# linyicheng1/keypoint_bench

Measured on AMD Instinct MI355X. Metric: image-pairs/sec (extract+NMS+BF-match, 640x480, top_k=1000), higher is better.
Workload: dtype f32

## Files before the change

### keypoint_bench_amd/csrc/alike.hip

```cpp
#include "conv_mfma.h"

namespace {

typedef _Float16 h8v __attribute__((ext_vector_type(8)));
typedef _Float16 h2v __attribute__((ext_vector_type(2)));
typedef float f32x4v __attribute__((ext_vector_type(4)));

__device__ __forceinline__ float relu(float v);

__device__ __forceinline__ void split4(const float4 v, uint2& hi, uint2& lo) { cm_split4(v, hi, lo); }

__device__ __forceinline__ void amax_commit(float lane_max, float* slots, int slot, int lane)
{
    const float m = cm_wave_max(lane_max);
    if (lane == 0) slots[slot] = m;
}

__global__ __launch_bounds__(256) void amax_reduce(const float* slots, int n, unsigned* out)
{
    __shared__ float s[4];
    const int b = blockIdx.x, tid = threadIdx.x;
    float m = 0.0f;
    for (int i = tid; i < n; i += 256) {
        const float v = slots[(size_t)b * n + i];
// ... 452 lines not shown
                    const float4 q = *reinterpret_cast<const float4*>(p + ((size_t)dy * Wr + dx) * CDS + c4 * 4);
                    v4.x = fmaxf(v4.x, q.x); v4.y = fmaxf(v4.y, q.y); v4.z = fmaxf(v4.z, q.z); v4.w = fmaxf(v4.w, q.w);
                }
            const float v[4] = {v4.x, v4.y, v4.z, v4.w};
#pragma unroll
            for (int c = 0; c < 4; ++c)
#pragma unroll
                for (int j = 0; j < 16; ++j) acc[j] = fmaf(v[c], dw[(c4 * 4 + c) * COUT + j], acc[j]);
        }
    }
    float* o = a.out + ((size_t)b * a.H * a.W + (size_t)gy * a.W + gx) * COUT + cg * 16;
#pragma unroll
    for (int q = 0; q < 4; ++q) {
        float4 v = make_float4(acc[4 * q], acc[4 * q + 1], acc[4 * q + 2], acc[4 * q + 3]);
        if (RELU) { v.x = relu(v.x); v.y = relu(v.y); v.z = relu(v.z); v.w = relu(v.w); }
        *reinterpret_cast<float4*>(o + 4 * q) = v;
    }
}

struct Block2Args {
    const float* p1;
    float* x2; float* a2; float* S2;
    float* p2;
    const uint4* w1pk;
    const uint4* w2pk;
    const uint4* wapk;
    const float* b1; const float* bsum; const float* wsg;
    int H, W;
    float inv_ws1, inv_ws2, inv_wsa, l1_c1, bmax_c1, l1_c2, l1_ds, bmax_sum;
    const unsigned* amax_x1;
    float* wmax_a2;
    int xcd_map;
};


__global__ __launch_bounds__(256, 4) void alike_block2(Block2Args a)
{
    constexpr int TH = 8, TW = 32, PH = TH + 4, PW = TW + 4, NP = PH * PW, MH = TH + 2, MW = TW + 2, NM = MH * MW;
    __shared__ __attribute__((aligned(16))) uint4 pin[2 * NP];
    __shared__ __attribute__((aligned(16))) uint4 mid[4 * NM];
    __shared__ __attribute__((aligned(16))) uint4 xs[4][2][2][16];
    __shared__ __attribute__((aligned(16))) uint4 zslot;
    const kpb_tile3 tile = kpb_xcd_tile(a.xcd_map);
    const int tid = threadIdx.x, lane = tid & 63, wv = tid >> 6, b = tile.z;
    const int ty0 = tile.y * TH, tx0 = tile.x * TW;
    const size_t P = (size_t)a.H * a.W;
    h8v w1h[3], w1l[3], w2h[5], w2l[5];
#pragma unroll
    for (int kb = 0; kb < 3; ++kb) { w1h[kb] = __builtin_bit_cast(h8v, a.w1pk[(kb * 2) * 64 + lane]); w1l[kb] = __builtin_bit_cast(h8v, a.w1pk[(kb * 2 + 1) * 64 + lane]); }
    const float4 b1v = *reinterpret_cast<const float4*>(a.b1 + 4 * (lane >> 4));
    const float4 bsum = *reinterpret_cast<const float4*>(a.bsum + 4 * (lane >> 4)), wsg = *reinterpret_cast<const float4*>(a.wsg + 4 * (lane >> 4));
    const float am_p = __uint_as_float(a.amax_x1[b]);
    const float bound1 = fmaf(am_p, a.l1_c1, a.bmax_c1);
    const int e1 = cm_exp_of(fmaxf(am_p, bound1));
    const int ex = cm_exp_of(fmaf(bound1, a.l1_c2, fmaf(am_p, a.l1_ds, a.bmax_sum)));
    const float sc1 = cm_scale_of(e1), un_c1s = a.inv_ws1, un_c2 = a.inv_ws2 * cm_unscale_of(e1);
    const bool edge = ty0 == 0 || tx0 == 0 || ty0 + TH >= a.H || tx0 + TW >= a.W;
    const float scx = cm_scale_of(ex), un_a = a.inv_wsa * cm_unscale_of(ex);
    {
        const float* in = a.p1 + (size_t)b * P * 8;
        constexpr int PER = (NP * 2 + 255) / 256;
        float4 ld[PER];
        unsigned okm = 0;
#pragma unroll
        for (int k = 0; k < PER; ++k) {
            const int i = min(tid + 256 * k, NP * 2 - 1);
            const int pos = i >> 1, q = i & 1;
            const int y = pos / PW, x = pos - y * PW;
            const int gy = ty0 - 2 + y, gx = tx0 - 2 + x;
            if (gy >= 0 && gy < a.H && gx >= 0 && gx < a.W) okm |= 1u << k;
            ld[k] = *reinterpret_cast<const float4*>(in + ((size_t)min(max(gy, 0), a.H - 1) * a.W + min(max(gx, 0), a.W - 1)) * 8 + 4 * q);
        }
#pragma unroll
        for (int k = 0; k < PER; ++k) {
            const int i = tid + 256 * k;
            const int pos = i >> 1, q = i & 1;
            float4 v = ((okm >> k) & 1u) ? ld[k] : make_float4(0.f, 0.f, 0.f, 0.f);
            v.x *= sc1; v.y *= sc1; v.z *= sc1; v.w *= sc1;
            uint2 hi, lo;
            split4(v, hi, lo);
            if (i < NP * 2) {
                uint2* d = reinterpret_cast<uint2*>(&pin[pos]) + q;
                d[0] = hi;
                d[2 * NP] = lo;
            }
        }
        if (tid == 0) zslot = make_uint4(0u, 0u, 0u, 0u);
    }
    __syncthreads();
    const int px = lane & 15, g = lane >> 4;
    const uint4* zp = &zslot;
    {
        float4 bias1 = b1v;
        bias1.x *= sc1; bias1.y *= sc1; bias1.z *= sc1; bias1.w *= sc1;
        uint2* midh = reinterpret_cast<uint2*>(mid);
        static_assert((2 * MH) % 4 == 0, "alike_block2: the regular conv1 groups split evenly over the four waves");
        {
            const int xl = 16 * (wv & 1) + px, y0 = wv >> 1;
            const int gxl = tx0 - 1 + xl;
            const bool xin = gxl >= 0 && gxl < a.W;
            const float unm = xin ? un_c1s : 0.0f;
            const float4 bm = xin ? bias1 : make_float4(0.f, 0.f, 0.f, 0.f);
            const bool has2 = 8 + g < 9;
            const uint4* q0 = &pin[(y0 + g / 3) * PW + xl + g % 3];
            const uint4* q1 = &pin[(y0 + (4 + g) / 3) * PW + xl + (4 + g) % 3];
            const uint4* q2 = has2 ? &pin[(y0 + 2) * PW + xl + 2] : zp;
            const int st2 = has2 ? 2 * PW : 0, lo2 = has2 ? NP : 0;
            int h8 = (((g >> 1) * NM + y0 * MW + xl) << 1) + (g & 1);
            constexpr int NIT = 2 * MH / 4;
            h8v i0h = __builtin_bit_cast(h8v, q0[0]), i0l = __builtin_bit_cast(h8v, q0[NP]);
            h8v i1h = __builtin_bit_cast(h8v, q1[0]), i1l = __builtin_bit_cast(h8v, q1[NP]);
            h8v i2h = __builtin_bit_cast(h8v, q2[0]), i2l = __builtin_bit_cast(h8v, q2[lo2]);
#pragma unroll 1
            for (int it = 0; it < NIT; ++it, h8 += 4 * MW) {
                f32x4v acc = {0.f, 0.f, 0.f, 0.f};
                __builtin_amdgcn_sched_barrier(0);
                acc = __builtin_amdgcn_mfma_f32_16x16x32_f16(w1h[0], i0l, acc, 0, 0, 0);
                acc = __builtin_amdgcn_mfma_f32_16x16x32_f16(w1l[0], i0h, acc, 0, 0, 0);
                acc = __builtin_amdgcn_mfma_f32_16x16x32_f16(w1h[0], i0h, acc, 0, 0, 0);
                acc = __builtin_amdgcn_mfma_f32_16x16x32_f16(w1h[1], i1l, acc, 0, 0, 0);
                acc = __builtin_amdgcn_mfma_f32_16x16x32_f16(w1l[1], i1h, acc, 0, 0, 0);
                acc = __builtin_amdgcn_mfma_f32_16x16x32_f16(w1h[1], i1h, acc, 0, 0, 0);
                acc = __builtin_amdgcn_mfma_f32_16x16x32_f16(w1h[2], i2l, acc, 0, 0, 0);
                acc = __builtin_amdgcn_mfma_f32_16x16x32_f16(w1l[2], i2h, acc, 0, 0, 0);
                acc = __builtin_amdgcn_mfma_f32_16x16x32_f16(w1h[2], i2h, acc, 0, 0, 0);
                __builtin_amdgcn_sched_barrier(0);
                if (it + 1 < NIT) {
                    q0 += 2 * PW; q1 += 2 * PW; q2 += st2;
                    i0h = __builtin_bit_cast(h8v, q0[0]); i0l = __builtin_bit_cast(h8v, q0[NP]);
                    i1h = __builtin_bit_cast(h8v, q1[0]); i1l = __builtin_bit_cast(h8v, q1[NP]);
                    i2h = __builtin_bit_cast(h8v, q2[0]); i2l = __builtin_bit_cast(h8v, q2[lo2]);
                }
                __builtin_amdgcn_sched_barrier(0);
                const bool yin = (unsigned)(ty0 - 1 + y0 + 2 * it) < (unsigned)a.H;
                float4 v = make_float4(0.f, 0.f, 0.f, 0.f);
                if (yin) v = make_float4(relu(fmaf(acc[0], unm, bm.x)), relu(fmaf(acc[1], unm, bm.y)), relu(fmaf(acc[2], unm, bm.z)), relu(fmaf(acc[3], unm, bm.w)));
                uint2 hi, lo;
                split4(v, hi, lo);
                midh[h8] = hi;
                midh[h8 + 4 * NM] = lo;
            }
        }
        if (wv < 2) {
            const int gi = 2 * MH + wv;
            const int k = 16 * (gi - 2 * MH) + px;
            const int y = k >> 1, x = 32 + (k & 1);
            const int my = min(y, MH - 1);
            f32x4v acc = {0.f, 0.f, 0.f, 0.f};
#pragma unroll
            for (int kb = 0; kb < 3; ++kb) {
                const int tap = 4 * kb + g;
                const bool has = tap < 9;
                const uint4* ph = has ? &pin[(my + tap / 3) * PW + x + tap % 3] : zp;
                const h8v ihi = __builtin_bit_cast(h8v, ph[0]);
                const h8v ilo = __builtin_bit_cast(h8v, has ? ph[NP] : zp[0]);
                acc = __builtin_amdgcn_mfma_f32_16x16x32_f16(w1h[kb], ilo, acc, 0, 0, 0);
                acc = __builtin_amdgcn_mfma_f32_16x16x32_f16(w1l[kb], ihi, acc, 0, 0, 0);
                acc = __builtin_amdgcn_mfma_f32_16x16x32_f16(w1h[kb], ihi, acc, 0, 0, 0);
            }
            const int gy = ty0 - 1 + y, gx = tx0 - 1 + x;
            const bool inside = gy >= 0 && gy < a.H && gx >= 0 && gx < a.W;
            float4 v = make_float4(relu(fmaf(acc[0], un_c1s, bias1.x)), relu(fmaf(acc[1], un_c1s, bias1.y)), relu(fmaf(acc[2], un_c1s, bias1.z)), relu(fmaf(acc[3], un_c1s, bias1.w)));
            if (edge && !inside) v = make_float4(0.f, 0.f, 0.f, 0.f);
            uint2 hi, lo;
            split4(v, hi, lo);
            if (y < MH) {
                const int h8 = (((g >> 1) * NM + y * MW + x) << 1) + (g & 1);
                midh[h8] = hi;
                midh[h8 + 4 * NM] = lo;
            }
        }
    }
    __builtin_amdgcn_sched_barrier(0);
#pragma unroll
    for (int kb = 0; kb < 5; ++kb) { w2h[kb] = __builtin_bit_cast(h8v, a.w2pk[(kb * 2) * 64 + lane]); w2l[kb] = __builtin_bit_cast(h8v, a.w2pk[(kb * 2 + 1) * 64 + lane]); }
    const h8v wah = __builtin_bit_cast(h8v, a.wapk[lane]), wal = __builtin_bit_cast(h8v, a.wapk[64 + lane]);
    __syncthreads();
    float* x2 = a.x2 + (size_t)b * P * 16;
    float* a2 = a.a2 + (size_t)b * P * 16;
    float* S2 = a.S2 + (size_t)b * P;
    uint2* xh = reinterpret_cast<uint2*>(&xs[wv][0][0][0]);
    float4 pm = make_float4(0.f, 0.f, 0.f, 0.f);
    float amx = 0.0f;
#pragma unroll 1
    for (int k4 = 0; k4 < 4; ++k4) {
        const int row = 4 * (wv >> 1) + k4, col0 = (wv & 1) * 16;
        const int mbase = row * MW + col0 + px;
        f32x4v acc = {0.f, 0.f, 0.f, 0.f};
        h8v ihi[5], ilo[5];
        auto fetch = [&](int kb) {
            const int kidx = 4 * kb + g;
            const uint4* ph;
            int lo_off;
            if (kidx < 18) { const int tap = kidx >> 1; ph = &mid[(kidx & 1) * NM + mbase + (tap / 3) * MW + tap % 3]; lo_off = 2 * NM; }
            else if (kidx == 18) { ph = &pin[(row + 2) * PW + col0 + px + 2]; lo_off = NP; }
            else { ph = zp; lo_off = 0; }
            ihi[kb] = __builtin_bit_cast(h8v, ph[0]);
            ilo[kb] = __builtin_bit_cast(h8v, ph[lo_off]);
        };
        auto mm = [&](int kb) {
            acc = __builtin_amdgcn_mfma_f32_16x16x32_f16(w2h[kb], ilo[kb], acc, 0, 0, 0);
            acc = __builtin_amdgcn_mfma_f32_16x16x32_f16(w2l[kb], ihi[kb], acc, 0, 0, 0);
            acc = __builtin_amdgcn_mfma_f32_16x16x32_f16(w2h[kb], ihi[kb], acc, 0, 0, 0);
        };
        fetch(0); fetch(1); fetch(2);
        __builtin_amdgcn_sched_barrier(0);
        mm(0); mm(1);
        __builtin_amdgcn_sched_barrier(0);
        fetch(3); fetch(4);
        __builtin_amdgcn_sched_barrier(0);
        mm(2);
        __builtin_amdgcn_sched_barrier(0);
        mm(3); mm(4);
        const int gy = ty0 + row, gx = tx0 + col0 + px;
        const bool ok = gy < a.H && gx < a.W;
        const float4 v = make_float4(relu(fmaf(acc[0], un_c2, bsum.x)), relu(fmaf(acc[1], un_c2, bsum.y)), relu(fmaf(acc[2], un_c2, bsum.z)), relu(fmaf(acc[3], un_c2, bsum.w)));
        if (ok && !a.p2) *reinterpret_cast<float4*>(x2 + ((size_t)gy * a.W + gx) * 16 + 4 * g) = v;
        pm = make_float4(kpb_pmax(pm.x, v.x), kpb_pmax(pm.y, v.y), kpb_pmax(pm.z, v.z), kpb_pmax(pm.w, v.w));
        {
            uint2 hi, lo;
            split4(make_float4(v.x * scx, v.y * scx, v.z * scx, v.w * scx), hi, lo);
            const int h8 = (((g >> 1) * 16 + px) << 1) + (g & 1);
            xh[h8] = hi;
            xh[h8 + 64] = lo;
        }
        f32x4v ag = {0.f, 0.f, 0.f, 0.f};
        {
            const uint4* ph = g < 2 ? &xs[wv][0][g][px] : zp;
            const h8v ihi = __builtin_bit_cast(h8v, ph[0]);
            const h8v ilo = __builtin_bit_cast(h8v, g < 2 ? ph[32] : zp[0]);
            ag = __builtin_amdgcn_mfma_f32_16x16x32_f16(wah, ilo, ag, 0, 0, 0);
            ag = __builtin_amdgcn_mfma_f32_16x16x32_f16(wal, ihi, ag, 0, 0, 0);
            ag = __builtin_amdgcn_mfma_f32_16x16x32_f16(wah, ihi, ag, 0, 0, 0);
        }
        const float4 av = make_float4(relu(ag[0] * un_a), relu(ag[1] * un_a), relu(ag[2] * un_a), relu(ag[3] * un_a));
        if (ok) {
            *reinterpret_cast<float4*>(a2 + ((size_t)gy * a.W + gx) * 16 + 4 * g) = av;
            amx = kpb_pmax(kpb_pmax(amx, kpb_pmax(av.x, av.y)), kpb_pmax(av.z, av.w));
        }
        float sg = fmaf(av.w, wsg.w, fmaf(av.z, wsg.z, fmaf(av.y, wsg.y, av.x * wsg.x)));
        sg = kpb_sum16(sg);
        sg = kpb_sum32(sg);
        if (g == 0 && ok) S2[(size_t)gy * a.W + gx] = sg;
    }
    if (a.p2) {
        pm.x = kpb_pmax(pm.x, kpb_xor1(pm.x)); pm.y = kpb_pmax(pm.y, kpb_xor1(pm.y));
        pm.z = kpb_pmax(pm.z, kpb_xor1(pm.z)); pm.w = kpb_pmax(pm.w, kpb_xor1(pm.w));
        pm.x = kpb_pmax(pm.x, kpb_xor2(pm.x)); pm.y = kpb_pmax(pm.y, kpb_xor2(pm.y));
        pm.z = kpb_pmax(pm.z, kpb_xor2(pm.z)); pm.w = kpb_pmax(pm.w, kpb_xor2(pm.w));
        const int gy = ty0 + 4 * (wv >> 1), gx = tx0 + (wv & 1) * 16 + px;
        if ((px & 3) == 0 && gy < a.H && gx < a.W)
            *reinterpret_cast<float4*>(a.p2 + (size_t)b * (P / 16) * 16 + ((size_t)(gy >> 2) * (a.W >> 2) + (gx >> 2)) * 16 + 4 * g) = pm;
    }
    amax_commit(amx, a.wmax_a2, ((b * gridDim.y + tile.y) * gridDim.x + tile.x) * 4 + wv, lane);
}

std::vector<float> pack_1x1_h16(const float* w, float scale)
{
    return pack_lanes_h16(1, [&](int, int l, int j) {
        const int n = l & 15, g = l >> 4;
        return g < 2 ? w[n * 16 + 8 * g + j] * scale : 0.0f;
    });
}

std::vector<float> pack_h16(const float* w, int CIN, const float* ds_w, float scale)
{
    const int OCT = CIN / 8, NK = 9 * OCT + (ds_w ? 1 : 0), KB = (NK + 3) / 4;
    return pack_lanes_h16(KB, [&](int kb, int l, int j) {
        const int n = l & 15, g = l >> 4, kidx = 4 * kb + g;
        float v = 0.0f;
        if (kidx < 9 * OCT) { const int tap = kidx / OCT, o = kidx - tap * OCT; v = w[((size_t)n * CIN + 8 * o + j) * 9 + tap]; }
        else if (ds_w && kidx == 9 * OCT) v = ds_w[n * 8 + j];
        return v * scale;
    });
}

// ... 35 lines not shown
    if (STAGE_IN) {
        const int ln = threadIdx.x & 63;
        const size_t pw = (size_t)bx * 256 + (threadIdx.x >> 6) * 64;
        float4 ld[CIN / 4];
#pragma unroll
        for (int i = 0; i < CIN / 4; ++i) {
            const int j = ln + 64 * i, px = j / (CIN / 4);
            ld[i] = pw + px < npix ? *reinterpret_cast<const float4*>(in + pw * CIN + 4 * (size_t)j) : make_float4(0.f, 0.f, 0.f, 0.f);
        }
#pragma unroll
        for (int i = 0; i < CIN / 4; ++i) {
            const int j = ln + 64 * i, px = j / (CIN / 4), q = j - px * (CIN / 4);
            *reinterpret_cast<float4*>(wreg + px * XP + 4 * q) = ld[i];
        }
        x = wreg + ln * XP;
    }
#pragma unroll 2
    for (int c4 = 0; c4 < CIN / 4; ++c4) {
        const float4 v4 = *reinterpret_cast<const float4*>(x + c4 * 4);
        const float v[4] = {v4.x, v4.y, v4.z, v4.w};
#pragma unroll
        for (int c = 0; c < 4; ++c)
#pragma unroll
            for (int j = 0; j < 16; ++j) acc[j] = fmaf(v[c], w[(c4 * 4 + c) * 16 + j], acc[j]);
    }
    float sg = 0.0f;
#pragma unroll
    for (int j = 0; j < 16; ++j) { acc[j] = relu(acc[j]); sg = fmaf(acc[j], wsg[j], sg); }
    if (live) {
        float* o = out + p * 16;
#pragma unroll
        for (int q = 0; q < 4; ++q)
            *reinterpret_cast<float4*>(o + 4 * q) = make_float4(acc[4 * q], acc[4 * q + 1], acc[4 * q + 2], acc[4 * q + 3]);
        smap[p] = sg;
    }
    if (E) {
        const int lane = threadIdx.x & 63, wv = threadIdx.x >> 6;
        float* st = wreg;
        const size_t p0 = (size_t)bx * 256 + wv * 64;
        float4 r[17];
#pragma unroll
        for (int q = 0; q < 16; ++q) {
            r[q] = make_float4(0.f, 0.f, 0.f, 0.f);
#pragma unroll
            for (int c = 0; c < 16; ++c) {
                const float* wr = wproj + c * 64 + 4 * q;
                r[q].x = fmaf(acc[c], wr[0], r[q].x); r[q].y = fmaf(acc[c], wr[1], r[q].y);
                r[q].z = fmaf(acc[c], wr[2], r[q].z); r[q].w = fmaf(acc[c], wr[3], r[q].w);
            }
        }
        r[16] = make_float4(sg, 0.f, 0.f, 0.f);
        for (int g = 0; g < 4; ++g) {
            if ((lane >> 4) == g) {
                float* e = st + (lane & 15) * ESTRIDE;
#pragma unroll
                for (int q = 0; q < 17; ++q) *reinterpret_cast<float4*>(e + 4 * q) = r[q];
            }
            const size_t base = p0 + 16 * g;
            for (int j = lane; j < 16 * (ESTRIDE / 4); j += 64)
                if (base + j / (ESTRIDE / 4) < npix)
                    *reinterpret_cast<float4*>(E + base * ESTRIDE + 4 * j) = *reinterpret_cast<const float4*>(st + 4 * j);
        }
    }
}

template <int CIN>
__global__ __launch_bounds__(256) void conv1x1_relu(const float* __restrict__ in, float* __restrict__ out, const float* __restrict__ w,
// ... 954 lines not shown
#pragma unroll
            for (int k = 0; k < 3; ++k) ds[r * (GP_TW * 3) + lane * 3 + k] = __fdiv_rn(1.0f, 1.0f + expf(-z[k]));
        }
    }
    if (!a.desc) return;
    __builtin_amdgcn_wave_barrier();
    const int vw = min(GP_TW, W - tx0) * 3;
#pragma unroll
    for (int k = 0; k < GP_RPT * GP_TW * 3 / 4 / 64; ++k) {
        const int f = k * 64 + lane, r = f / (GP_TW * 3 / 4), c4 = (f - r * (GP_TW * 3 / 4)) * 4;
        if (c4 < vw && yw + r < H)
            *reinterpret_cast<float4*>(a.desc + (img + (size_t)(yw + r) * W + tx0) * 3 + c4) = *reinterpret_cast<const float4*>(ds + r * (GP_TW * 3) + c4);
    }
}

}

namespace {

struct AlikeBlock1 : kpb_net {
    float* x1 = nullptr;
    struct { const float *w1, *b1, *w2, *b2; const uint4 *w1pk, *w2pk; float inv_ws1, inv_ws2, l1_c1, bmax_c1; } k1 = {};
    struct B1Bufs { float *p1, *wmax_x1; unsigned* amax_x1; };
    static int b1_waves(int H, int W) { return cdiv(W, B1_TW) * cdiv(H, B1H_TH) * 4; }
    void block1(const float* img_dev, int batch, int H, int W, const B1Bufs& b);
};

struct AlikeTrunk : AlikeBlock1 {
    float *a2 = nullptr, *a3 = nullptr, *a4 = nullptr;
    struct { const uint4 *w1pk, *w2pk, *wapk; const float *b1, *bsum; float inv_ws1, inv_ws2, inv_wsa, l1_c1, bmax_c1, l1_c2, l1_ds, bmax_sum; } k2 = {};
    struct Res { const float *w1, *b1, *w2, *b2, *dsw, *dsb, *w1h, *b1h, *w2p, *b2p; float un1, un2; const char *prof1, *prof2; } blk[5] = {};
    struct { const float *agg[5], *whT, *wsc; const uint4 *wh16, *a1h16; float l1_agg1, inv_ws_h, inv_wa; } kh = {};
    struct Maps { float *S2, *S3, *S4, *E3, *E4; unsigned *amax_x1, *amax_a2; };
    int trunk(const float* img_dev, int batch, int H, int W, bool dense, Maps& m);
};

struct AlikeNet : AlikeTrunk {
    int forward(const float* img_dev, int batch, int H_, int W_, float* score_out_dev, float* desc_out_dev) override;
    int desc_at(const float* pts_dev, int pts_cols, int max_n, const int32_t* n_dev, float* out_dev) override;
};

void repack3x3(const float* w, int co, int ci, std::vector<float>& out)
{
    out.resize((size_t)9 * ci * co);
    for (int o = 0; o < co; ++o)
        for (int c = 0; c < ci; ++c)
            for (int k = 0; k < 9; ++k) out[((size_t)k * ci + c) * co + o] = w[((size_t)o * ci + c) * 9 + k];
}
void transpose(const float* w, int co, int ci, std::vector<float>& out)
{
    out.resize((size_t)ci * co);
    for (int o = 0; o < co; ++o)
        for (int c = 0; c < ci; ++c) out[(size_t)c * co + o] = w[(size_t)o * ci + c];
}
float l1_rows(const float* w, int co, int per)
{
    float m = 0.0f;
    for (int o = 0; o < co; ++o) {
        double s = 0.0;
        for (int i = 0; i < per; ++i) s += std::fabs((double)w[(size_t)o * per + i]);
        m = std::max(m, (float)(s * (1.0 + 1e-6)));
    }
    return m;
}
float max_abs(const float* b, int n)
{
    float m = 0.0f;
// ... 16 lines not shown
__global__ __launch_bounds__(256) void maxpool4_nhwc(const float* __restrict__ in, float* __restrict__ out, int Ho, int Wo, int C)
{
    const int C4 = C / 4;
    const size_t i = (size_t)blockIdx.x * 256 + threadIdx.x, b = blockIdx.y;
    if (i >= (size_t)Ho * Wo * C4) return;
    const int c = (int)(i % C4) * 4;
    const size_t pix = i / C4;
    const int y = (int)(pix / Wo), x = (int)(pix - (size_t)y * Wo);
    const float* s = in + ((b * 4 * Ho + 4 * y) * (size_t)(4 * Wo) + 4 * x) * C + c;
    float4 m = *reinterpret_cast<const float4*>(s);
#pragma unroll
    for (int py = 0; py < 4; ++py)
#pragma unroll
        for (int px = 0; px < 4; ++px) {
            if (py == 0 && px == 0) continue;
            const float4 v = *reinterpret_cast<const float4*>(s + ((size_t)py * 4 * Wo + px) * C);
            m.x = fmaxf(m.x, v.x); m.y = fmaxf(m.y, v.y); m.z = fmaxf(m.z, v.z); m.w = fmaxf(m.w, v.w);
        }
    *reinterpret_cast<float4*>(out + ((b * Ho + y) * (size_t)Wo + x) * C + c) = m;
}

void AlikeBlock1::block1(const float* img_dev, int batch, int H, int W, const B1Bufs& b)
{
    hipStream_t st = ctx->stream;
    Block1Args b1{img_dev, x1, b.p1, k1.w1, k1.b1, k1.w2, k1.b2, H, W};
    if (conv_mfma_use_h16()) {
        Block1HArgs hb{b1, k1.w1pk, k1.w2pk, k1.inv_ws1, k1.inv_ws2, k1.l1_c1, k1.bmax_c1, b.wmax_x1, 0};
        KPB_LAUNCH(ctx, "alike_block1", alike_block1_h, dim3(cdiv(W, B1_TW), cdiv(H, B1H_TH), batch), dim3(256), 0, st, hb);
        KPB_LAUNCH(ctx, "amax_reduce", amax_reduce, dim3(batch), dim3(256), 0, st, b.wmax_x1, b1_waves(H, W), b.amax_x1);
    } else
        KPB_LAUNCH(ctx, "alike_block1", alike_block1, dim3(cdiv(W, B1_TW), cdiv(H, B1_TH), batch), dim3(256), 0, st, b1);
}

int AlikeTrunk::trunk(const float* img_dev, int batch, int H, int W, bool dense, Maps& mo)
{
    const size_t P = (size_t)H * W, B = batch;
    const bool h16 = conv_mfma_use_h16();
    const bool fused = h16 && batch >= 16 && ctx->alike_coarse_fused;
    const int nw1 = b1_waves(H, W), nw2 = cdiv(W / 2, 32) * cdiv(H / 2, 8) * 4;
    const size_t n_2 = B * (P / 4) * 16, n_3 = B * (P / 64) * 32, n_4 = B * (P / 1024) * 64;
    float *p1, *t2, *x2, *t3, *x3, *t4, *x4, *r3, *r4, *t3r3, *t4r4, *p2, *p3, *S2, *S3, *S4, *E3, *E4, *wmax_x1, *wmax_a2;
    unsigned *amax_x1, *amax_a2;
    if (int rc = kpb_carve(ctx, act, [&](Arena& a) {
            auto f32 = [&](size_t n) { return h16 ? nullptr : a.take(n); };
            auto f16 = [&](size_t n) { return h16 ? a.take(n) : nullptr; };
            x1 = a.take(B * P * 8);
            p1 = a.take(B * (P / 4) * 8);
            t2 = f32(n_2); x2 = f32(n_2); a2 = a.take(n_2);
            t3 = f32(n_3); x3 = fused ? nullptr : a.take(n_3); a3 = a.take(B * (P / 64) * 16);
            t4 = f32(n_4); x4 = fused ? nullptr : a.take(n_4); a4 = a.take(B * (P / 1024) * 16);
            r3 = f32(n_3); r4 = f32(n_4);
            t3r3 = f16(2 * n_3);
            t4r4 = f16(2 * n_4);
            p2 = f16(n_3 / 2);
            p3 = h16 && batch >= 16 ? a.take(n_4 / 2) : nullptr;
            S2 = a.take(B * (P / 4)); S3 = a.take(B * (P / 64)); S4 = a.take(B * (P / 1024));
            E3 = dense ? a.take(B * (P / 64) * ESTRIDE) : nullptr;
            E4 = dense ? a.take(B * (P / 1024) * ESTRIDE) : nullptr;
            amax_x1 = h16 ? a.take<unsigned>(B) : nullptr;
            amax_a2 = h16 ? a.take<unsigned>(B) : nullptr;
            wmax_x1 = f16(B * nw1);
            wmax_a2 = f16(B * nw2);
        }))
        return rc;
    this->B = batch; this->H = H; this->W = W;
    hipStream_t st = ctx->stream;

    block1(img_dev, batch, H, W, B1Bufs{p1, wmax_x1, amax_x1});
    ConvArgs c;
    if (h16) {
        Block2Args b2{p1, x2, a2, S2, p2, k2.w1pk, k2.w2pk, k2.wapk, k2.b1, k2.bsum, kh.wsc + 16, H / 2, W / 2,
                      k2.inv_ws1, k2.inv_ws2, k2.inv_wsa, k2.l1_c1, k2.bmax_c1, k2.l1_c2, k2.l1_ds, k2.bmax_sum, amax_x1, wmax_a2, 1};
        KPB_LAUNCH(ctx, "alike_block2", alike_block2, dim3(cdiv(W / 2, 32), cdiv(H / 2, 8), batch), dim3(256), 0, st, b2);
        KPB_LAUNCH(ctx, "amax_reduce", amax_reduce, dim3(batch), dim3(256), 0, st, wmax_a2, nw2, amax_a2);
        auto block_h = [&](const Res& r, const float* in, float* tr, float* xo, int cin, int cout, int Hi, int Wi, bool prepooled, int gi = 0, float* ao = nullptr,
                           float* So = nullptr, float* Eo = nullptr, float* pool = nullptr) {
            ConvM m{.in = in, .out = tr, .wp = r.w1h, .bias = r.b1h, .Hi = prepooled ? Hi / 4 : Hi, .Wi = prepooled ? Wi / 4 : Wi,
                    .H = Hi / 4, .W = Wi / 4, .CIN = cin, .COUT = 2 * cout, .NCH = 1, .relu = 2, .nblk = cout / 32, .istride = cin, .ostride = 2 * cout,
                    .unscale = r.un1, .relu_nt = cout / 32};
            auto launch = [&](const char* prof, const CmForm& f, const ConvM& cm) {
                return launch_conv_mfma_h<CM_C16, CM_C32, CM_C32_1T, CM_C16_LAT, CM_C32_LAT, CM_P4_LAT, CM_B3C2_TAIL, CM_B4C2_TAIL>(ctx, prof, f, cm, batch); };
            if (batch < 16 && !prepooled) m.nblk = 2 * cout / 32;
            const CmForm f1 = !prepooled ? CM_P4_LAT : batch < 16 ? CM_C16_LAT : cin == 32 ? CM_C32 : CM_C16;
            if (int rc = launch(r.prof1, f1, m)) return rc;
            ConvM c2{.in = tr, .out = xo, .wp = r.w2p, .bias = r.b2p, .res = tr + cout, .Hi = Hi / 4, .Wi = Wi / 4,
                     .H = Hi / 4, .W = Wi / 4, .CIN = cout, .COUT = cout, .NCH = cout / 32, .nblk = batch < 16 ? cout / 32 : 1, .istride = 2 * cout,
                     .ostride = cout, .unscale = r.un2, .rstride = 2 * cout};
            if (ao) {
                c2.tl_w = kh.agg[gi]; c2.tl_wsg = kh.wsc + 16 * (gi - 1); c2.tl_wproj = kh.whT + 16 * (gi - 1) * 64;
                c2.tl_agg = ao; c2.tl_smap = So; c2.tl_E = Eo; c2.tl_pool = pool;
                return launch(r.prof2, pool ? CM_B3C2_TAIL : CM_B4C2_TAIL, c2);
            }
            return launch(r.prof2, batch < 16 ? CM_C32_LAT : cout == 32 ? CM_C32_1T : CM_C32, c2);
        };
        if (fused) {
            if (int rc = block_h(blk[3], p2, t3r3, nullptr, 16, 32, H / 2, W / 2, true, 3, a3, S3, E3, p3)) return rc;
            if (int rc = block_h(blk[4], p3, t4r4, nullptr, 32, 64, H / 8, W / 8, true, 4, a4, S4, E4)) return rc;
        } else if (int rc = block_h(blk[3], p2, t3r3, x3, 16, 32, H / 2, W / 2, true))
            return rc;
        else if (batch >= 16) {
            KPB_LAUNCH(ctx, "maxpool4_x3", maxpool4_nhwc, dim3((unsigned)(((size_t)(H / 32) * (W / 32) * 8 + 255) / 256), batch), dim3(256), 0, st, x3, p3, H / 32, W / 32, 32);
            if (int rc = block_h(blk[4], p3, t4r4, x4, 32, 64, H / 8, W / 8, true)) return rc;
        } else if (int rc = block_h(blk[4], x3, t4r4, x4, 32, 64, H / 8, W / 8, false))
            return rc;
    } else {
        auto conv2 = [&](const Res& r, const float* in, float* out, const float* res, int h, int w, int c) {
// ... 7 lines not shown
        c = ConvArgs{t2, x2, blk[2].w2, blk[2].b2, p1, blk[2].dsw, blk[2].dsb, nullptr, H / 2, W / 2};
        launch_conv<16, 16, 1, true, 8, 1>(ctx, "conv3x3_b2c2", st, c, batch);
        c = ConvArgs{x2, t3, blk[3].w1, blk[3].b1, nullptr, blk[3].dsw, blk[3].dsb, r3, H / 8, W / 8};
        launch_conv<16, 32, 4, false, 4, 1, true, 16>(ctx, "conv3x3_b3c1", st, c, batch);
        if (int rc = conv2(blk[3], t3, x3, r3, H / 8, W / 8, 32)) return rc;
        c = ConvArgs{x3, t4, blk[4].w1, blk[4].b1, nullptr, blk[4].dsw, blk[4].dsb, r4, H / 32, W / 32};
        launch_conv<32, 64, 4, false, 4, 1, true, 16>(ctx, "conv3x3_b4c1", st, c, batch);
        if (int rc = conv2(blk[4], t4, x4, r4, H / 32, W / 32, 64)) return rc;
        KPB_LAUNCH(ctx, "conv1x1_agg2", conv1x1_relu<16>, dim3((unsigned)((B * P / 4 + 255) / 256)), dim3(256), 0, st, x2, a2, kh.agg[2], kh.wsc + 16, S2, B * P / 4, nullptr, nullptr);
    }
    if (fused)
        ;
    else if (batch < 16) {
        const AggArgs g3{x3, a3, kh.agg[3], kh.wsc + 32, S3, B * P / 64, kh.whT + 32 * 64, E3};
        const AggArgs g4{x4, a4, kh.agg[4], kh.wsc + 48, S4, B * P / 1024, kh.whT + 48 * 64, E4};
        const unsigned nb3 = (unsigned)((B * P / 64 + 255) / 256), nb4 = (unsigned)((B * P / 1024 + 255) / 256);
        KPB_LAUNCH(ctx, "conv1x1_agg34", conv1x1_relu_34, dim3(nb3 + nb4), dim3(256), 0, st, g3, g4, nb3);
    } else {
        KPB_LAUNCH(ctx, "conv1x1_agg3", conv1x1_relu<32>, dim3((unsigned)((B * P / 64 + 255) / 256)), dim3(256), 0, st, x3, a3, kh.agg[3], kh.wsc + 32, S3, B * P / 64, kh.whT + 32 * 64, E3);
        KPB_LAUNCH(ctx, "conv1x1_agg4", conv1x1_relu<64>, dim3((unsigned)((B * P / 1024 + 255) / 256)), dim3(256), 0, st, x4, a4, kh.agg[4], kh.wsc + 48, S4, B * P / 1024, kh.whT + 48 * 64, E4);
    }
    mo = Maps{S2, S3, S4, E3, E4, amax_x1, amax_a2};
    return KPB_OK;
}

int AlikeNet::forward(const float* img_dev, int batch, int H_, int W_, float* score_out_dev, float* desc_out_dev)
{
    if ((H_ % 32) || (W_ % 32))
        return kpb_fail(ctx, KPB_E_INVALID, "kpb_net_forward: ALIKE needs H and W multiples of 32 (got %dx%d)", H_, W_);
    const int H = H_, W = W_;
    const bool h16 = conv_mfma_use_h16();
    const bool dense = desc_out_dev != nullptr;
    Maps m;
    if (int rc = trunk(img_dev, batch, H, W, dense, m)) return rc;
    float *S2 = m.S2, *S3 = m.S3, *S4 = m.S4, *E3 = m.E3, *E4 = m.E4;
    unsigned *amax_x1 = m.amax_x1, *amax_a2 = m.amax_a2;
    hipStream_t st = ctx->stream;
    if (dense) {
        HybArgs hy{x1, a2, E3, E4, kh.agg[1], kh.whT, kh.wsc, score_out_dev, desc_out_dev, H, W, amax_x1, amax_a2, 0.f, 1.f, 1.f, nullptr, 1.f};
        const int work4 = cdiv(H, 4) * cdiv(W / 32, SEG_TILES);
        if (h16) {
            hy.l1_agg1 = kh.l1_agg1; hy.inv_ws_h = kh.inv_ws_h; hy.ws_h = 1.0f / hy.inv_ws_h;
            hy.a1h16 = kh.a1h16; hy.inv_wa = kh.inv_wa;
            if (!hp_ring_rows_ok(H, H / 2, HP_A2R) || !hp_ring_rows_ok(H, H / 8, HP_ER) || !hp_ring_rows_ok(H, H / 32, HP_ER))
                return kpb_fail(ctx, KPB_E_UNSUPPORTED, "alike head: the LDS rings cannot hold the source rows of %d row groups at height %d", HP_LA + 1, H);
            const int bands_ = cdiv(W / 32, HP_TILES), groups_ = H / 4;
            const int hp = std::max(2, std::min(30, (int)(((long long)bands_ * groups_ * batch) / 1536)));
            KPB_LAUNCH(ctx, "alike_head_dense", alike_head_f16p, dim3(cdiv(W / 32, HP_TILES) * cdiv(H / 4, hp), batch), dim3(256), 0, st, hy,
                       kh.wh16, hp);
        } else
            KPB_LAUNCH(ctx, "alike_head_dense", alike_head_hyb, dim3(work4, batch), dim3(256), 0, st, hy);
    } else {
        LinArgs la{x1, S2, S3, S4, kh.agg[1], kh.wsc, score_out_dev, H, W,
                   (float)(H / 2 - 1) / (float)(H - 1), (float)(W / 2 - 1) / (float)(W - 1), (float)(H / 8 - 1) / (float)(H - 1), (float)(W / 8 - 1) / (float)(W - 1),
                   (float)(H / 32 - 1) / (float)(H - 1), (float)(W / 32 - 1) / (float)(W - 1)};
        KPB_LAUNCH(ctx, "alike_head_score", alike_score_lin, dim3(cdiv(H * W, 256), batch), dim3(256), 0, st, la);
    }
    KPB_HIP(ctx, hipGetLastError());
    return KPB_OK;
}

int AlikeNet::desc_at(const float* pts_dev, int pts_cols, int max_n, const int32_t* n_dev, float* out_dev)
{
    if (B == 0) return kpb_fail(ctx, KPB_E_INVALID, "kpb_net_desc_at: no forward has run");
    const int kpw = (long long)B * max_n >= 32768 ? 8 : 1;
    DescAtArgs a{HeadArgs{x1, a2, a3, a4, kh.agg[1], kh.whT, kh.wsc, nullptr, nullptr, H, W}, pts_dev, n_dev, out_dev, pts_cols, max_n, kpw};
    KPB_LAUNCH(ctx, "alike_desc_at", alike_desc_at, dim3(cdiv(max_n, 4 * kpw), B), dim3(256), 0, ctx->stream, a);
// ... 132 lines not shown
    trunk_stage(bl, ws, net.get());
    net->kh.l1_agg1 = l1_rows(bl.get("agg1.w", {dim / 4, c1}), 16, 8);
    const float* hw = bl.get("head.w", {dim + 1, dim});
    transpose(hw, 64, 64, tmp); ws.put(tmp, &net->kh.whT);
    ws.put_raw(hw + 64 * 64, 64, &net->kh.wsc);
    float hmax = 0.0f;
    for (int o = 0; o < 64; ++o) for (int cc = 0; cc < 32; ++cc) hmax = std::max(hmax, std::fabs(hw[o * 64 + cc]));
    const float* a1w = bl.get("agg1.w", {dim / 4, c1});
    const float sh = weight_scale_h(&hmax, 1), sa1 = weight_scale_h(a1w, 16 * 8);
    net->kh.inv_ws_h = 1.0f / sh; net->kh.inv_wa = 1.0f / sa1;
    ws.put(pack_head_h16(hw, sh), &net->kh.wh16);
    ws.put(pack_agg1_h16(a1w, sa1), &net->kh.a1h16);
    if (int rc = ws.upload(ctx, &net->wdev)) return rc;
    *out = net.release();
    return KPB_OK;
}

namespace {

struct EdgePointNet : AlikeTrunk {
    struct { const float *wsc, *tab, *tabb; } ke = {};
    int forward(const float* img_dev, int batch, int H_, int W_, float* score_out_dev, float* desc_out_dev) override;
};

int EdgePointNet::forward(const float* img_dev, int batch, int H_, int W_, float* score_out_dev, float* desc_out_dev)
{
    if ((H_ % 32) || (W_ % 32))
        return kpb_fail(ctx, KPB_E_INVALID, "kpb_net_forward: EdgePoint needs H and W multiples of 32 (got %dx%d)", H_, W_);
    const size_t npix = (size_t)batch * H_ * W_;
    const size_t nb_score = (npix + 256 * EPS_PPL - 1) / (256 * EPS_PPL);
    if (npix / 64 > 0xffffffffu || nb_score > 0x7fffffffu)
        return kpb_fail(ctx, KPB_E_UNSUPPORTED, "kpb_net_forward: EdgePoint: %d images of %dx%d exceed the head kernels' index range", batch, H_, W_);
    Maps m;
    if (int rc = trunk(img_dev, batch, H_, W_, false, m)) return rc;
    hipStream_t st = ctx->stream;
    KPB_LAUNCH(ctx, "edgepoint_score", edgepoint_score, dim3((unsigned)nb_score), dim3(256), 0, st, x1, score_out_dev, ke.wsc, npix);
    if (desc_out_dev) {
        const unsigned nc = (unsigned)(npix / 64);
        EpDescArgs d{x1, a2, a3, a4, ke.wsc, ke.tab, ke.tabb, kh.whT, desc_out_dev, H_, W_, nc};
        KPB_LAUNCH(ctx, "edgepoint_desc", edgepoint_desc, dim3(std::min((nc + 15u) / 16u, 2048u)), dim3(256), 0, st, d);
    }
    KPB_HIP(ctx, hipGetLastError());
    return KPB_OK;
}

}

int edgepoint_create(kpb_ctx* ctx, const KpbwBlob& bl, kpb_net** out)
{
    const uint32_t q = dim / 4;
    if (const char* n = first_missing(bl, {{"head.w", {dim, dim}}, {"score.w", {q}}, {"score.b", {1}}, {"d8.w", {q, q}}, {"d8.b", {q}}, {"d4.w", {q, q}}, {"d4.b", {q}},
                                           {"ct4.w", {q, q, 4, 4}}, {"ct4.b", {q}}}))
        return kpb_fail(ctx, KPB_E_WEIGHTS, "kpb_net_create: tensor %s missing or not EdgePoint shaped "
                        "(this build supports c1..c4 = 8,16,32,64, dim = 64, single head)", n);
    auto net = std::make_unique<EdgePointNet>();
    net->ctx = ctx; net->arch = KPB_ARCH_EDGEPOINT; net->dim = dim; net->desc_div = 8;
    WeightStage ws;
    std::vector<float> tmp;
    trunk_stage(bl, ws, net.get());
    ws.put(std::vector<float>(64, 0.0f), &net->kh.wsc);
    transpose(bl.get("head.w", {dim, dim}), 64, 64, tmp); ws.put(tmp, &net->kh.whT);
    {
        const float *w1 = bl.get("agg1.w", {q, c1}), *wsr = bl.get("score.w", {q});
        tmp.assign(EP_WBIAS + 1, 0.0f);
        for (int c = 0; c < 16; ++c) {
            for (int k = 0; k < 8; ++k) tmp[c * EP_WROW + k] = w1[c * 8 + k];
            tmp[c * EP_WROW + 8] = wsr[c];
// ... 139 lines not shown
```

### keypoint_bench_amd/csrc/conv_mfma.h

```cpp
#pragma once
#include <type_traits>
#include "net.h"

#include <algorithm>
#include <cmath>
#include <cstring>

namespace {

typedef float f32x16 __attribute__((ext_vector_type(16)));

__device__ __forceinline__ float relu(float v) { return fmaxf(v, 0.0f); }

struct ConvM {
    const float* in = nullptr;
    float* out = nullptr;
    const float* wp = nullptr;
    const float* bias = nullptr;
    const float* xf = nullptr;
    const int* active = nullptr;
    const float* res = nullptr;
    int Hi = 0, Wi = 0, H = 0, W = 0, CIN = 0, COUT = 0, NCH = 0, relu = 0, nblk = 0;
    int istride = 0, ostride = 0, ooff = 0;
    float unscale = 1.0f;
// ... 242 lines not shown

template <int CT>
__device__ __forceinline__ void cm_tail_agg(const float* x, float* strip, const float* w_ , const float* wsg_ ,
                                            const float* wproj_ , float* __restrict__ out, float* __restrict__ smap, float* __restrict__ E,
                                            const size_t (&row_pix)[4], const int (&ncol)[4], int lane, int half)
{
    typedef const __attribute__((address_space(4))) float* cfp;
    const cfp w = (cfp)w_, wsg = (cfp)wsg_, wproj = (cfp)wproj_;
    float acc[16];
#pragma unroll
    for (int j = 0; j < 16; ++j) acc[j] = 0.0f;
#pragma unroll 2
    for (int c4 = 0; c4 < CT / 4; ++c4) {
        const float4 v4 = *reinterpret_cast<const float4*>(x + c4 * 4);
        const float v[4] = {v4.x, v4.y, v4.z, v4.w};
#pragma unroll
        for (int c = 0; c < 4; ++c)
#pragma unroll
            for (int j = 0; j < 16; ++j) acc[j] = fmaf(v[c], w[(c4 * 4 + c) * 16 + j], acc[j]);
    }
    float sg = 0.0f;
#pragma unroll
    for (int j = 0; j < 16; ++j) { acc[j] = relu(acc[j]); sg = fmaf(acc[j], wsg[j], sg); }
    const int g_own = lane >> 4, col = lane & 15;
    size_t pix = 0; bool live = false;
#pragma unroll
    for (int g = 0; g < 4; ++g)
        if (g == g_own) { pix = row_pix[g] + col; live = col < ncol[g]; }
    if (live && half == 0) {
        float* o = out + pix * 16;
#pragma unroll
        for (int q = 0; q < 4; ++q)
            *reinterpret_cast<float4*>(o + 4 * q) = make_float4(acc[4 * q], acc[4 * q + 1], acc[4 * q + 2], acc[4 * q + 3]);
        smap[pix] = sg;
    }
    if (!E) return;
#pragma unroll
    for (int rnd = 0; rnd < 2; ++rnd) {
        const int q0 = 8 * half + 4 * rnd;
        float4 r[4];
#pragma unroll
        for (int k = 0; k < 4; ++k) {
            r[k] = make_float4(0.f, 0.f, 0.f, 0.f);
#pragma unroll
            for (int c = 0; c < 16; ++c) {
                const cfp wr = wproj + c * 64 + 4 * (q0 + k);
                r[k].x = fmaf(acc[c], wr[0], r[k].x); r[k].y = fmaf(acc[c], wr[1], r[k].y);
                r[k].z = fmaf(acc[c], wr[2], r[k].z); r[k].w = fmaf(acc[c], wr[3], r[k].w);
            }
        }
#pragma unroll
        for (int g = 0; g < 4; ++g) {
            if (g_own == g) {
#pragma unroll
                for (int k = 0; k < 4; ++k) *reinterpret_cast<float4*>(strip + col * 16 + 4 * k) = r[k];
            }
            if ((lane >> 2) < ncol[g])
                *reinterpret_cast<float4*>(E + (row_pix[g] + (lane >> 2)) * CM_ESTRIDE + 4 * (q0 + (lane & 3))) = *reinterpret_cast<const float4*>(strip + 4 * lane);
        }
    }
    if (live && half == 1) *reinterpret_cast<float4*>(E + pix * CM_ESTRIDE + 64) = make_float4(sg, 0.f, 0.f, 0.f);
}

template <CmForm F>
__global__ __launch_bounds__(256, F.waves()) void conv_mfma_h(ConvM a)
{
    constexpr int KS = F.ks, S = F.s, CC = F.cc, NTB = F.ntb, MT = F.mt, PF = F.pf, WN = F.wn, DIL = F.dil;
// ... 882 lines not shown
```

Measured before the change: 15950.

## Template alike_block2 to skip unused x2 and score-map outputs

alike_block2 becomes a template on whether it writes the x2 map and the per-pixel score map S2. The trunk now allocates and writes S2/S3/S4 only when the share path needs them, which is when no dense descriptors are requested. The x2 store is removed at compile time. Indexing is simplified to a 32-bit pixel offset with column-only bounds, and the conv2 tap fetch now uses a strength-reduced pointer, which relies on new checks that H and W are multiples of 32. Downstream smap writes are guarded by null checks.

Result: no change. 15920 (-0.2%).

```diff
diff --git a/keypoint_bench_amd/csrc/alike.hip b/keypoint_bench_amd/csrc/alike.hip
--- a/keypoint_bench_amd/csrc/alike.hip
+++ b/keypoint_bench_amd/csrc/alike.hip
@@ -508,8 +508,9 @@
     float* wmax_a2;
     int xcd_map;
 };
-
-
+struct B2Form { bool share, x2; };
+
+template <B2Form F>
 __global__ __launch_bounds__(256, 4) void alike_block2(Block2Args a)
 {
     constexpr int TH = 8, TW = 32, PH = TH + 4, PW = TW + 4, NP = PH * PW, MH = TH + 2, MW = TW + 2, NM = MH * MW;
@@ -566,6 +567,7 @@
     __syncthreads();
     const int px = lane & 15, g = lane >> 4;
     const uint4* zp = &zslot;
+    const int wvs = __builtin_amdgcn_readfirstlane(wv);
     {
         float4 bias1 = b1v;
         bias1.x *= sc1; bias1.y *= sc1; bias1.z *= sc1; bias1.w *= sc1;
@@ -608,7 +610,7 @@
                     i2h = __builtin_bit_cast(h8v, q2[0]); i2l = __builtin_bit_cast(h8v, q2[lo2]);
                 }
                 __builtin_amdgcn_sched_barrier(0);
-                const bool yin = (unsigned)(ty0 - 1 + y0 + 2 * it) < (unsigned)a.H;
+                const bool yin = (unsigned)(ty0 - 1 + (wvs >> 1) + 2 * it) < (unsigned)a.H;
                 float4 v = make_float4(0.f, 0.f, 0.f, 0.f);
                 if (yin) v = make_float4(relu(fmaf(acc[0], unm, bm.x)), relu(fmaf(acc[1], unm, bm.y)), relu(fmaf(acc[2], unm, bm.z)), relu(fmaf(acc[3], unm, bm.w)));
                 uint2 hi, lo;
@@ -652,27 +654,33 @@
     for (int kb = 0; kb < 5; ++kb) { w2h[kb] = __builtin_bit_cast(h8v, a.w2pk[(kb * 2) * 64 + lane]); w2l[kb] = __builtin_bit_cast(h8v, a.w2pk[(kb * 2 + 1) * 64 + lane]); }
     const h8v wah = __builtin_bit_cast(h8v, a.wapk[lane]), wal = __builtin_bit_cast(h8v, a.wapk[64 + lane]);
     __syncthreads();
-    float* x2 = a.x2 + (size_t)b * P * 16;
-    float* a2 = a.a2 + (size_t)b * P * 16;
-    float* S2 = a.S2 + (size_t)b * P;
+    char* x2 = F.x2 ? reinterpret_cast<char*>(a.x2 + (size_t)b * P * 16) : nullptr;
+    char* a2 = reinterpret_cast<char*>(a.a2 + (size_t)b * P * 16);
+    char* S2 = F.share ? reinterpret_cast<char*>(a.S2 + (size_t)b * P) : nullptr;
     uint2* xh = reinterpret_cast<uint2*>(&xs[wv][0][0][0]);
     float4 pm = make_float4(0.f, 0.f, 0.f, 0.f);
     float amx = 0.0f;
+    const int row0 = 4 * (wvs >> 1), col0 = (wvs & 1) * 16;
+    const bool colin = tx0 + col0 < a.W;
+    unsigned pixo = (unsigned)((ty0 + row0) * a.W + tx0 + col0 + px);
+    const uint4* q4 = g < 2 ? &mid[g * NM + (row0 + 2) * MW + col0 + px + 2] : g == 2 ? &pin[(row0 + 2) * PW + col0 + px + 2] : zp;
+    const int st4 = g < 2 ? MW : g == 2 ? PW : 0, lo4 = g < 2 ? 2 * NM : g == 2 ? NP : 0;
 #pragma unroll 1
-    for (int k4 = 0; k4 < 4; ++k4) {
-        const int row = 4 * (wv >> 1) + k4, col0 = (wv & 1) * 16;
-        const int mbase = row * MW + col0 + px;
+    for (int k4 = 0; k4 < 4; ++k4, q4 += st4, pixo += (unsigned)a.W) {
+        const int mbase = (row0 + k4) * MW + col0 + px;
         f32x4v acc = {0.f, 0.f, 0.f, 0.f};
         h8v ihi[5], ilo[5];
         auto fetch = [&](int kb) {
-            const int kidx = 4 * kb + g;
-            const uint4* ph;
-            int lo_off;
-            if (kidx < 18) { const int tap = kidx >> 1; ph = &mid[(kidx & 1) * NM + mbase + (tap / 3) * MW + tap % 3]; lo_off = 2 * NM; }
-            else if (kidx == 18) { ph = &pin[(row + 2) * PW + col0 + px + 2]; lo_off = NP; }
-            else { ph = zp; lo_off = 0; }
+            if (kb == 4) {
+                ihi[kb] = __builtin_bit_cast(h8v, q4[0]);
+                ilo[kb] = __builtin_bit_cast(h8v, q4[lo4]);
+                return;
+            }
+            const int kidx = 4 * kb + g, tap = kidx >> 1;
+            const int ty = (tap * 11) >> 5;
+            const uint4* ph = &mid[(kidx & 1) * NM + mbase + ty * MW + tap - 3 * ty];
             ihi[kb] = __builtin_bit_cast(h8v, ph[0]);
-            ilo[kb] = __builtin_bit_cast(h8v, ph[lo_off]);
+            ilo[kb] = __builtin_bit_cast(h8v, ph[2 * NM]);
         };
         auto mm = [&](int kb) {
             acc = __builtin_amdgcn_mfma_f32_16x16x32_f16(w2h[kb], ilo[kb], acc, 0, 0, 0);
@@ -688,10 +696,9 @@
         mm(2);
         __builtin_amdgcn_sched_barrier(0);
         mm(3); mm(4);
-        const int gy = ty0 + row, gx = tx0 + col0 + px;
-        const bool ok = gy < a.H && gx < a.W;
+        const unsigned vo = pixo * 64u + 16u * g;
         const float4 v = make_float4(relu(fmaf(acc[0], un_c2, bsum.x)), relu(fmaf(acc[1], un_c2, bsum.y)), relu(fmaf(acc[2], un_c2, bsum.z)), relu(fmaf(acc[3], un_c2, bsum.w)));
-        if (ok && !a.p2) *reinterpret_cast<float4*>(x2 + ((size_t)gy * a.W + gx) * 16 + 4 * g) = v;
+        if (F.x2 && colin) *reinterpret_cast<float4*>(x2 + vo) = v;
         pm = make_float4(kpb_pmax(pm.x, v.x), kpb_pmax(pm.y, v.y), kpb_pmax(pm.z, v.z), kpb_pmax(pm.w, v.w));
         {
             uint2 hi, lo;
@@ -710,14 +717,16 @@
             ag = __builtin_amdgcn_mfma_f32_16x16x32_f16(wah, ihi, ag, 0, 0, 0);
         }
         const float4 av = make_float4(relu(ag[0] * un_a), relu(ag[1] * un_a), relu(ag[2] * un_a), relu(ag[3] * un_a));
-        if (ok) {
-            *reinterpret_cast<float4*>(a2 + ((size_t)gy * a.W + gx) * 16 + 4 * g) = av;
+        if (colin) {
+            *reinterpret_cast<float4*>(a2 + vo) = av;
             amx = kpb_pmax(kpb_pmax(amx, kpb_pmax(av.x, av.y)), kpb_pmax(av.z, av.w));
         }
-        float sg = fmaf(av.w, wsg.w, fmaf(av.z, wsg.z, fmaf(av.y, wsg.y, av.x * wsg.x)));
-        sg = kpb_sum16(sg);
-        sg = kpb_sum32(sg);
-        if (g == 0 && ok) S2[(size_t)gy * a.W + gx] = sg;
+        if (F.share) {
+            float sg = fmaf(av.w, wsg.w, fmaf(av.z, wsg.z, fmaf(av.y, wsg.y, av.x * wsg.x)));
+            sg = kpb_sum16(sg);
+            sg = kpb_sum32(sg);
+            if (g == 0 && colin) *reinterpret_cast<float*>(S2 + pixo * 4u) = sg;
+        }
     }
     if (a.p2) {
         pm.x = kpb_pmax(pm.x, kpb_xor1(pm.x)); pm.y = kpb_pmax(pm.y, kpb_xor1(pm.y));
@@ -819,7 +828,7 @@
 #pragma unroll
         for (int q = 0; q < 4; ++q)
             *reinterpret_cast<float4*>(o + 4 * q) = make_float4(acc[4 * q], acc[4 * q + 1], acc[4 * q + 2], acc[4 * q + 3]);
-        smap[p] = sg;
+        if (smap) smap[p] = sg;
     }
     if (E) {
         const int lane = threadIdx.x & 63, wv = threadIdx.x >> 6;
@@ -1840,7 +1849,7 @@
     struct Res { const float *w1, *b1, *w2, *b2, *dsw, *dsb, *w1h, *b1h, *w2p, *b2p; float un1, un2; const char *prof1, *prof2; } blk[5] = {};
     struct { const float *agg[5], *whT, *wsc; const uint4 *wh16, *a1h16; float l1_agg1, inv_ws_h, inv_wa; } kh = {};
     struct Maps { float *S2, *S3, *S4, *E3, *E4; unsigned *amax_x1, *amax_a2; };
-    int trunk(const float* img_dev, int batch, int H, int W, bool dense, Maps& m);
+    int trunk(const float* img_dev, int batch, int H, int W, bool dense, bool share, Maps& m);
 };
 
 struct AlikeNet : AlikeTrunk {
@@ -1923,8 +1932,12 @@
         KPB_LAUNCH(ctx, "alike_block1", alike_block1, dim3(cdiv(W, B1_TW), cdiv(H, B1_TH), batch), dim3(256), 0, st, b1);
 }
 
-int AlikeTrunk::trunk(const float* img_dev, int batch, int H, int W, bool dense, Maps& mo)
-{
+int AlikeTrunk::trunk(const float* img_dev, int batch, int H, int W, bool dense, bool share, Maps& mo)
+{
+    if ((H % 32) || (W % 32))
+        return kpb_fail(ctx, KPB_E_INVALID, "alike trunk: H and W must be multiples of 32 (got %dx%d)", H, W);
+    if ((size_t)(H / 2) * (W / 2) * 64 >= ((size_t)1 << 31))
+        return kpb_fail(ctx, KPB_E_UNSUPPORTED, "alike trunk: a %dx%d image's half-resolution map exceeds 2^31 bytes", H, W);
     const size_t P = (size_t)H * W, B = batch;
     const bool h16 = conv_mfma_use_h16();
     const bool fused = h16 && batch >= 16 && ctx->alike_coarse_fused;
@@ -1945,7 +1958,7 @@
             t4r4 = f16(2 * n_4);
             p2 = f16(n_3 / 2);
             p3 = h16 && batch >= 16 ? a.take(n_4 / 2) : nullptr;
-            S2 = a.take(B * (P / 4)); S3 = a.take(B * (P / 64)); S4 = a.take(B * (P / 1024));
+            S2 = share ? a.take(B * (P / 4)) : nullptr; S3 = share ? a.take(B * (P / 64)) : nullptr; S4 = share ? a.take(B * (P / 1024)) : nullptr;
             E3 = dense ? a.take(B * (P / 64) * ESTRIDE) : nullptr;
             E4 = dense ? a.take(B * (P / 1024) * ESTRIDE) : nullptr;
             amax_x1 = h16 ? a.take<unsigned>(B) : nullptr;
@@ -1962,7 +1975,8 @@
     if (h16) {
         Block2Args b2{p1, x2, a2, S2, p2, k2.w1pk, k2.w2pk, k2.wapk, k2.b1, k2.bsum, kh.wsc + 16, H / 2, W / 2,
                       k2.inv_ws1, k2.inv_ws2, k2.inv_wsa, k2.l1_c1, k2.bmax_c1, k2.l1_c2, k2.l1_ds, k2.bmax_sum, amax_x1, wmax_a2, 1};
-        KPB_LAUNCH(ctx, "alike_block2", alike_block2, dim3(cdiv(W / 2, 32), cdiv(H / 2, 8), batch), dim3(256), 0, st, b2);
+        if (share) KPB_LAUNCH(ctx, "alike_block2", (alike_block2<B2Form{true, false}>), dim3(cdiv(W / 2, 32), cdiv(H / 2, 8), batch), dim3(256), 0, st, b2);
+        else KPB_LAUNCH(ctx, "alike_block2", (alike_block2<B2Form{false, false}>), dim3(cdiv(W / 2, 32), cdiv(H / 2, 8), batch), dim3(256), 0, st, b2);
         KPB_LAUNCH(ctx, "amax_reduce", amax_reduce, dim3(batch), dim3(256), 0, st, wmax_a2, nw2, amax_a2);
         auto block_h = [&](const Res& r, const float* in, float* tr, float* xo, int cin, int cout, int Hi, int Wi, bool prepooled, int gi = 0, float* ao = nullptr,
                            float* So = nullptr, float* Eo = nullptr, float* pool = nullptr) {
@@ -2036,7 +2050,7 @@
     const bool h16 = conv_mfma_use_h16();
     const bool dense = desc_out_dev != nullptr;
     Maps m;
-    if (int rc = trunk(img_dev, batch, H, W, dense, m)) return rc;
+    if (int rc = trunk(img_dev, batch, H, W, dense, !dense, m)) return rc;
     float *S2 = m.S2, *S3 = m.S3, *S4 = m.S4, *E3 = m.E3, *E4 = m.E4;
     unsigned *amax_x1 = m.amax_x1, *amax_a2 = m.amax_a2;
     hipStream_t st = ctx->stream;
@@ -2235,7 +2249,7 @@
     if (npix / 64 > 0xffffffffu || nb_score > 0x7fffffffu)
         return kpb_fail(ctx, KPB_E_UNSUPPORTED, "kpb_net_forward: EdgePoint: %d images of %dx%d exceed the head kernels' index range", batch, H_, W_);
     Maps m;
-    if (int rc = trunk(img_dev, batch, H_, W_, false, m)) return rc;
+    if (int rc = trunk(img_dev, batch, H_, W_, false, false, m)) return rc;
     hipStream_t st = ctx->stream;
     KPB_LAUNCH(ctx, "edgepoint_score", edgepoint_score, dim3((unsigned)nb_score), dim3(256), 0, st, x1, score_out_dev, ke.wsc, npix);
     if (desc_out_dev) {
diff --git a/keypoint_bench_amd/csrc/conv_mfma.h b/keypoint_bench_amd/csrc/conv_mfma.h
--- a/keypoint_bench_amd/csrc/conv_mfma.h
+++ b/keypoint_bench_amd/csrc/conv_mfma.h
@@ -298,7 +298,7 @@
 #pragma unroll
         for (int q = 0; q < 4; ++q)
             *reinterpret_cast<float4*>(o + 4 * q) = make_float4(acc[4 * q], acc[4 * q + 1], acc[4 * q + 2], acc[4 * q + 3]);
-        smap[pix] = sg;
+        if (smap) smap[pix] = sg;
     }
     if (!E) return;
 #pragma unroll
```
